# widdowquinn/pyani

Hardware: AMD Instinct MI355X
Metric: genome-pairs/sec (ordered pairs) + wall-clock for the N x N ANIm grid: nucmer --mum + delta-filter -1 + parse_delta equivalent per ordered pair, genomes resident in HBM; vs the CPU path on this box's host cores (higher is better)
Workload: dtype u32 packed DP words (score << 17 | state << 15 | errors), i64 lengths, f64 identity

## Files before the change

### pyani_amd/csrc/pg_nucmer_diag.h

```cpp
#pragma once
#include <stdint.h>
#include "pg_nucmer_core.h"

namespace pgd {
using namespace pgn;

template <int DPL> struct DiagRegs { uint32_t X[DPL], D[DPL], I[DPL], mw[DPL]; };

PG_HD uint32_t rev16_fields(uint32_t x) {
#if defined(__HIP_DEVICE_COMPILE__)
  x = __brev(x);
#else
  x = ((x >> 1) & 0x55555555u) | ((x & 0x55555555u) << 1);
  x = ((x >> 2) & 0x33333333u) | ((x & 0x33333333u) << 2);
  x = ((x >> 4) & 0x0F0F0F0Fu) | ((x & 0x0F0F0F0Fu) << 4);
  x = ((x >> 8) & 0x00FF00FFu) | ((x & 0x00FF00FFu) << 8);
  x = (x >> 16) | (x << 16);
#endif
  return ((x & 0x55555555u) << 1) | ((x >> 1) & 0x55555555u);
}
PG_HD uint32_t spread16(uint32_t m) {
  m &= 0xFFFFu;
  m = (m | (m << 8)) & 0x00FF00FFu;
  m = (m | (m << 4)) & 0x0F0F0F0Fu;
  m = (m | (m << 2)) & 0x33333333u;
  m = (m | (m << 1)) & 0x55555555u;
  return m;
}

struct DiagRelabel { uint32_t mask, st_insert, st_match; };
template <int DPL, int PAR, bool NORM = false>
PG_HD uint32_t diag_lane_edge(const DiagRegs<DPL>& T) {
  constexpr int32_t RISE = NORM && PAR == 0 ? GOOD_SCORE : 0;
  const uint32_t c = w_gap(PAR == 0 ? T.D[DPL - 1] : T.I[0], CONT_GAP_SCORE - RISE), x = w_gap(PAR == 0 ? T.X[DPL - 1] : T.X[0], OPEN_GAP_SCORE - RISE);
  return c > x ? c : x;
}
template <int DPL, int PAR, bool TRACK, bool NORM = false>
PG_HD void diag_lane_step(DiagRegs<DPL>& T, uint32_t nbM, uint32_t g0, uint32_t glo, uint32_t gspan, const DiagRelabel& rel,
                          uint32_t& key, uint32_t& keyw) {
  key = 0u; keyw = 0u;
  const uint32_t gofs = g0 - glo;
  constexpr int32_t RISE = NORM && PAR == 0 ? GOOD_SCORE : 0;
#if defined(__HIP_DEVICE_COMPILE__)
#pragma unroll
#endif
  for (int s = PAR; s < DPL; s += 2) {
    uint32_t dm, im;
    if (s == 0) dm = nbM;
    else { const uint32_t dc = w_gap(T.D[s - 1], CONT_GAP_SCORE - RISE), dx = w_gap(T.X[s - 1], OPEN_GAP_SCORE - RISE); dm = dc > dx ? dc : dx; }
    if (s == DPL - 1) im = nbM;
    else { const uint32_t ic = w_gap(T.I[s + 1], CONT_GAP_SCORE - RISE), ix = w_gap(T.X[s + 1], OPEN_GAP_SCORE - RISE); im = ic > ix ? ic : ix; }
    const bool in = (uint32_t)(gofs + (uint32_t)s) <= gspan;
    const uint32_t mk = in ? rel.mask : 0u;
    const uint32_t d = dm & mk , i = s == DPL - 1 ? (im & mk) + rel.st_insert : (im & mk) | rel.st_insert;
    const uint32_t m = ((NORM ? w_step_norm(T.X[s], T.mw[s]) : w_step_window(T.X[s], T.mw[s])) & mk) | rel.st_match;
    T.mw[s] <<= 2;
    T.X[s] = w_max3(d, i, m); T.D[s] = d; T.I[s] = i;
    if (TRACK) {
      const uint32_t k = (T.X[s] & ~(W_ONE - 1u)) | (g0 + (uint32_t)s);
      if (k >= key) { key = k; keyw = T.X[s]; }
    }
  }
}
template <int DPL, int PAR>
PG_HD void diag_lane_key(const DiagRegs<DPL>& T, uint32_t g0, uint32_t& key, uint32_t& keyw) {
  key = 0u; keyw = 0u;
#if defined(__HIP_DEVICE_COMPILE__)
#pragma unroll
#endif
  for (int s = PAR; s < DPL; s += 2) {
    const uint32_t k = (T.X[s] & ~(W_ONE - 1u)) | (g0 + (uint32_t)s);
    if (k >= key) { key = k; keyw = T.X[s]; }
  }
}
template <int DPL, int PAR>
PG_HD uint32_t diag_lane_top(const DiagRegs<DPL>& T) {
  uint32_t top = 0u;
#if defined(__HIP_DEVICE_COMPILE__)
#pragma unroll
#endif
  for (int s = PAR; s < DPL; s += 2) top = T.X[s] > top ? T.X[s] : top;
  return top;
}
template <int DPL, int PAR>
PG_HD uint32_t diag_lane_alive(const DiagRegs<DPL>& T, uint32_t thr) {
  uint32_t bits = 0u;
  for (int s = PAR; s < DPL; s += 2) bits |= (T.X[s] >= thr ? 1u : 0u) << s;
  return bits;
}
template <int DPL, int PAR, bool NORM = false, bool CLEAN = false>
PG_HD void diag_lane_refill(DiagRegs<DPL>& T, uint64_t ca, uint32_t oka, uint64_t cb, uint32_t okb) {
  constexpr int e_last = ((DPL - 1) ^ PAR) & 1, e_0 = PAR & 1;
#if defined(__HIP_DEVICE_COMPILE__)
#pragma unroll
#endif
  for (int s = 0; s < DPL; ++s) {
    const int e_s = (s ^ PAR) & 1;
    const int oa = (DPL - 1 - s + e_s - e_last) / 2, ob = (s + e_s - e_0) / 2;
    const uint32_t a16 = (uint32_t)(ca >> (2 * oa)), b16 = (uint32_t)(cb >> (2 * ob));
    const uint32_t x = a16 ^ b16;
    const uint32_t eq = ~(x | (x >> 1)) & 0x55555555u;
    const uint32_t hit = CLEAN ? eq : eq & spread16((oka >> oa) & (okb >> ob));
    T.mw[s] = rev16_fields(NORM ? hit ^ 0x55555555u : hit) << 1;
  }
}
template <int DPL, int PAR>
PG_HD void diag_refill_origin(int32_t Dct, int32_t k0, int32_t& ia0, int32_t& jb0) {
  constexpr int e_last = ((DPL - 1) ^ PAR) & 1, e_0 = PAR & 1;
  const int32_t u = Dct - k0;
  ia0 = (u - (DPL - 1) + e_last) >> 1;
  jb0 = ((u + e_0) >> 1) + k0;
}

struct DiagCtl {
  int32_t N, M, NM;
  bool fwd, forced, optimal, banded;
  int32_t Dct, Dend;
  int32_t ga, gb;
  int32_t lo, hi;
  int32_t c1g, c2g;
  int32_t kming, kmaxg;
  int32_t shiftk;
  uint32_t high_f, high_w;
  uint32_t high_fw, thr_w;
  int32_t FinishCt, FinishG, FinishShift;
  uint32_t span_sum;
  int32_t wmax;
  int32_t next_refill;
  template <int DPL>
  PG_HD void init(int32_t N_, int32_t M_, unsigned m_o, int32_t band_w) {
    constexpr int32_t HALF = 32 * DPL;
    N = N_; M = M_; NM = N_ + M_;
    fwd = m_o & DIRECTION_BIT; forced = m_o & FORCED_BIT; optimal = m_o & OPTIMAL_BIT; banded = band_w >= 0;
    kming = (M - N < 0 ? M - N : 0) - band_w + HALF; kmaxg = (M - N > 0 ? M - N : 0) + band_w + HALF;
    Dct = 1; Dend = forced ? NM : (NM < BREAK_LEN ? NM : BREAK_LEN);
    ga = HALF - 1; gb = HALF + 1; lo = HALF; hi = HALF; shiftk = 0;
    c1g = 1 - 2 * N + HALF; c2g = 2 * M - 1 + HALF;
    high_f = 0u; high_w = 0u; FinishCt = 0; FinishG = HALF; FinishShift = 0;
    high_fw = 0u; thr_w = (0u - (uint32_t)MAX_DIFF) << SCORE_SHIFT;
    span_sum = 0u; wmax = 0; next_refill = 1;
  }
  template <bool FORCED>
  PG_HD int begin_step() {
    if (Dct > Dend) return 1;
    lo = ga > c1g ? ga : c1g; hi = gb < c2g ? gb : c2g;
    if (FORCED && banded) {
      if (lo < kming) lo = kming;
      if (hi > kmaxg) hi = kmaxg;
      if ((lo + Dct) & 1) ++lo;
      if ((hi + Dct) & 1) --hi;
    }
    return lo > hi ? 2 : 0;
  }
  template <bool FORCED>
  PG_HD bool begin_step_go() {
    lo = ga > c1g ? ga : c1g; hi = gb < c2g ? gb : c2g;
    if (FORCED && banded) {
      if (lo < kming) lo = kming;
      if (hi > kmaxg) hi = kmaxg;
      if ((lo + Dct) & 1) ++lo;
      if ((hi + Dct) & 1) --hi;
    }
    return ((Dend - Dct) | (hi - lo)) >= 0;
  }
  template <int DPL>
  PG_HD int32_t window_check() const {
    constexpr int32_t W = 64 * DPL, HALF = W / 2;
    if (lo >= 2 && hi <= W - 3) return 0;
    if (hi - lo + 5 > W) return INT32_MIN;
    int32_t n = ((lo + hi) / 2 - HALF) / DPL;
    if (n == 0) n = lo < 2 ? -1 : 1;
    if (lo - DPL * n < 2 || hi - DPL * n > W - 3) return INT32_MIN;
    return n;
  }
  template <int DPL>
  PG_HD void window_move(int32_t n) { window_shift(DPL * n); }
  PG_HD void window_shift(int32_t d) {
    shiftk += d; lo -= d; hi -= d; ga -= d; gb -= d; c1g -= d; c2g -= d; kming -= d; kmaxg -= d;
    next_refill = Dct;
  }
  template <bool WIDEST>
  PG_HD void note_cells() {
    span_sum += (uint32_t)(hi - lo);
    if (WIDEST) { const int32_t w = (hi - lo) / 2 + 1; if (w > wmax) wmax = w; }
  }
  PG_HD int32_t steps() const { return Dct - 1; }
  PG_HD unsigned long long cells_total() const { return (unsigned long long)(span_sum / 2u) + (unsigned long long)steps(); }
  PG_HD void update_best(uint32_t gk, uint32_t gw) {
    const uint32_t f = gk >> SCORE_SHIFT;
    if (f >= (high_fw >> SCORE_SHIFT)) {
      high_f = f; high_w = gw; high_fw = f << SCORE_SHIFT; thr_w = (f - (uint32_t)MAX_DIFF) << SCORE_SHIFT; FinishCt = Dct; FinishG = (int32_t)(gk & (W_ONE - 1u)); FinishShift = shiftk;
      Dend = Dct + BREAK_LEN < NM ? Dct + BREAK_LEN : NM;
    }
  }
  PG_HD uint32_t trim_threshold() const { return thr_w; }
  template <bool FORCED, bool NORM_EVEN = false>
  PG_HD void end_step(bool any, uint32_t gmin, uint32_t gmax) {
    if (FORCED) { ga = lo - 1; gb = hi + 1; }
    else if (any) { ga = (int32_t)gmin - 1; gb = (int32_t)gmax + 1; }
    else { ga = 0; gb = 1; Dend = -1; }
    ++Dct; ++c1g; --c2g;
    if (NORM_EVEN) { high_fw -= (uint32_t)GOOD_SCORE << SCORE_SHIFT; thr_w -= (uint32_t)GOOD_SCORE << SCORE_SHIFT; }
  }
  template <int DPL>
  PG_HD bool finish1(bool& reached, uint32_t& corner_slot, int32_t& FinishK) {
    constexpr int32_t HALF = 32 * DPL;
    reached = false;
    const int32_t last = Dct - 1;
    corner_slot = 0u;
    FinishK = FinishG - HALF + FinishShift;
    if (last == NM) {
      if (!optimal) { reached = true; FinishCt = NM; FinishK = M - N; corner_slot = (uint32_t)(M - N - shiftk + HALF); return true; }
      if (FinishCt == last) reached = true;
    }
    return false;
  }
  template <bool NORM = false>
  PG_HD void finish2(uint32_t fin_w, int32_t FinishK, int32_t Astart, int32_t Bstart, int32_t& Aend, int32_t& Bend, int32_t& errors, int32_t& score) const {
    const int32_t fi = (FinishCt - FinishK) / 2, fj = (FinishCt + FinishK) / 2;
    Aend = fwd ? Astart + fi - 1 : Astart - fi + 1;
    Bend = fwd ? Bstart + fj - 1 : Bstart - fj + 1;
    errors = (int32_t)w_errors(fin_w);
    score = NORM ? (int32_t)(fin_w >> SCORE_SHIFT) - (int32_t)NORM_BIAS + norm_offset(FinishCt) : w_score(fin_w);
  }
};

#if !defined(__HIP_DEVICE_COMPILE__)
template <int DPL, typename RefT, typename QryT>
struct DiagWaveEmu {
  static constexpr int W = 64 * DPL, HALF = W / 2;
  const RefT& R;
  const QryT& Q;
  long cells = 0, calls = 0, moves = 0, fails = 0;
  uint32_t last_cells = 0, last_wmax = 0;
  DiagRegs<DPL> T[64];
  template <int PAR, bool NORM>
  void refill(const DiagCtl& C, int32_t Astart, int32_t Bstart) {
    for (int l = 0; l < 64; ++l) {
      const int32_t k0 = DPL * l - HALF + C.shiftk;
      int32_t ia0, jb0;
      diag_refill_origin<DPL, PAR>(C.Dct, k0, ia0, jb0);
      uint64_t ca = 0, cb = 0; uint32_t oka = 0, okb = 0;
      for (int f = 0; f < 32; ++f) {
        const int64_t pa = C.fwd ? (int64_t)Astart + (ia0 + f) - 1 : (int64_t)Astart - (ia0 + f) + 1;
        const int64_t pb = C.fwd ? (int64_t)Bstart + (jb0 + f) - 1 : (int64_t)Bstart - (jb0 + f) + 1;
        if (R.clean(pa)) { ca |= (uint64_t)R.base(pa) << (2 * f); oka |= 1u << f; }
        if (Q.clean(pb)) { cb |= (uint64_t)Q.base(pb) << (2 * f); okb |= 1u << f; }
      }
      if ((oka & okb) == 0xFFFFFFFFu) diag_lane_refill<DPL, PAR, NORM, true>(T[l], ca, oka, cb, okb);
      else diag_lane_refill<DPL, PAR, NORM, false>(T[l], ca, oka, cb, okb);
    }
  }
  template <int PAR, bool FORCED>
  void step(DiagCtl& C) {
    uint32_t nbM[64], key[64], keyw[64];
    for (int l = 0; l < 64; ++l) {
      if (PAR == 0) nbM[l] = l > 0 ? diag_lane_edge<DPL, PAR, !FORCED>(T[l - 1]) : 0u;
      else nbM[l] = l < 63 ? diag_lane_edge<DPL, PAR, !FORCED>(T[l + 1]) : 0u;
    }
    for (int l = 0; l < 64; ++l)
      diag_lane_step<DPL, PAR, !FORCED, !FORCED>(T[l], nbM[l], (uint32_t)(DPL * l), (uint32_t)C.lo, (uint32_t)(C.hi - C.lo), DiagRelabel{~W_STATE, ST_INSERT, ST_MATCH}, key[l], keyw[l]);
    bool any = false; uint32_t gmin = 0, gmax = 0;
    if (!FORCED) {
      uint32_t gk = 0, gw = 0;
      for (int l = 0; l < 64; ++l) if (key[l] > gk) { gk = key[l]; gw = keyw[l]; }
      C.update_best(gk, gw);
      const uint32_t thr = C.trim_threshold();
      for (int l = 0; l < 64; ++l) {
        const uint32_t bits = diag_lane_alive<DPL, PAR>(T[l], thr);
        for (int s = PAR; s < DPL; s += 2)
          if ((bits >> s) & 1u) { const uint32_t g = (uint32_t)(DPL * l + s); if (!any) { gmin = g; any = true; } gmax = g; }
      }
    }
    C.template end_step<FORCED, !FORCED && PAR == 1>(any, gmin, gmax);
  }
  template <bool FORCED>
  bool run_(int32_t Astart, int32_t& Aend, int32_t Bstart, int32_t& Bend, unsigned m_o, int32_t band_w, int32_t& errors, int32_t& score, bool& reached) {
    DiagCtl C;
    const bool fwd = m_o & DIRECTION_BIT;
    C.template init<DPL>(fwd ? Aend - Astart + 1 : Astart - Aend + 1, fwd ? Bend - Bstart + 1 : Bstart - Bend + 1, m_o, band_w);
    for (int l = 0; l < 64; ++l) for (int s = 0; s < DPL; ++s) { T[l].X[s] = 0u; T[l].D[s] = 0u; T[l].I[s] = 0u; T[l].mw[s] = 0u; }
    T[HALF / DPL].X[0] = FORCED ? w_make(0, 0, ST_MATCH) : (NORM_BIAS << SCORE_SHIFT) | ST_MATCH;
    ++calls;
    for (;;) {
      if (C.template begin_step<FORCED>()) break;
      const int32_t n = C.template window_check<DPL>();
      if (n == INT32_MIN) { ++fails; return false; }
      if (n != 0) {
        DiagRegs<DPL> Z;
        for (int s = 0; s < DPL; ++s) { Z.X[s] = 0u; Z.D[s] = 0u; Z.I[s] = 0u; Z.mw[s] = 0u; }
        DiagRegs<DPL> U[64];
        for (int l = 0; l < 64; ++l) U[l] = (l + n >= 0 && l + n < 64) ? T[l + n] : Z;
        for (int l = 0; l < 64; ++l) T[l] = U[l];
        C.template window_move<DPL>(n);
        ++moves;
      }
      if (C.Dct == C.next_refill) { if (C.Dct & 1) refill<1, !FORCED>(C, Astart, Bstart); else refill<0, !FORCED>(C, Astart, Bstart); C.next_refill = C.Dct + 32; }
      C.template note_cells<true>();
      if (C.Dct & 1) step<1, FORCED>(C); else step<0, FORCED>(C);
    }
    uint32_t corner = 0, fin_w = C.high_w;
    int32_t FinishK = 0;
    if (C.template finish1<DPL>(reached, corner, FinishK)) fin_w = T[corner / DPL].X[corner % DPL];
    C.template finish2<!FORCED>(fin_w, FinishK, Astart, Bstart, Aend, Bend, errors, score);
    const unsigned long long nc = C.cells_total();
    cells += (long)nc;
    last_cells = nc > 0xFFFFFFFFull ? 0xFFFFFFFFu : (uint32_t)nc; last_wmax = (uint32_t)C.wmax;
    return true;
  }
  bool run(int32_t Astart, int32_t& Aend, int32_t Bstart, int32_t& Bend, unsigned m_o, int32_t band_w, int32_t& errors, int32_t& score, bool& reached) {
    return (m_o & FORCED_BIT) ? run_<true>(Astart, Aend, Bstart, Bend, m_o, band_w, errors, score, reached)
                              : run_<false>(Astart, Aend, Bstart, Bend, m_o, band_w, errors, score, reached);
  }
};
#endif

PG_HD bool diag_window_holds(int64_t span, int dpl) { return span <= 64 * (int64_t)dpl - 2 * (int64_t)dpl + 2; }
#if !defined(__HIP_DEVICE_COMPILE__)
template <typename RefT, typename QryT>
struct DiagWaveEngine {
  ScalarEngine<RefT, QryT> slow;
  DiagWaveEmu<2, RefT, QryT> e2;
  DiagWaveEmu<4, RefT, QryT> e4;
  DiagWaveEmu<6, RefT, QryT> e6;
  DiagWaveEmu<8, RefT, QryT> e8;
  DiagWaveEmu<12, RefT, QryT> e12;
  DiagWaveEmu<16, RefT, QryT> e16;
  DiagWaveEmu<24, RefT, QryT> e24;
  DiagWaveEmu<32, RefT, QryT> e32;
  long fallbacks = 0;
  void (*fallback_log)(int32_t N, int32_t M, unsigned m_o, int32_t band_w) = nullptr;
  DiagWaveEngine(const RefT& R, const QryT& Q, Cell* d0, Cell* d1, Cell* d2, int32_t cap)
      : slow{R, Q, d0, d1, d2, cap}, e2{R, Q}, e4{R, Q}, e6{R, Q}, e8{R, Q}, e12{R, Q}, e16{R, Q}, e24{R, Q}, e32{R, Q} {}
  bool gap_ready(int32_t, PnGap&) const { return false; }
  void piece(uint32_t, int32_t, int32_t, int32_t, int32_t, int32_t, int32_t, int32_t, unsigned) {}
  bool bwd_ready(int, PnBwd&) const { return false; }
  void bwd_key(int, int32_t, int32_t, int32_t, int32_t, unsigned) {}
  bool fwd_ready(int, PnFwd&) const { return false; }
  int32_t forced_errors(int32_t A0, int32_t A1, int32_t B0, int32_t B1, PnAln*) {
    int32_t err = 0, a = A1, b = B1;
    align(A0, a, B0, b, FORCED_FORWARD_ALIGN, err);
    return err;
  }
  bool shadowed(const Chain* chains, const PnAln* al, int from, int c, int32_t sA, int32_t eA, int32_t sB, int32_t eB) const {
    return PnScalarScans().shadowed(chains, al, from, c, sA, eA, sB, eB); }
  int shadow_first(const Chain* chains, const PnAln* al, int n_al, int c, int32_t sA, int32_t eA, int32_t sB, int32_t eB) const {
    return PnScalarScans().shadow_first(chains, al, n_al, c, sA, eA, sB, eB); }
  int reverse_target(const Chain* chains, const PnAln* al, int cura, int c, int32_t sA, int32_t sB, int32_t dist) const {
    return PnScalarScans().reverse_target(chains, al, cura, c, sA, sB, dist); }
  int forward_target(const Chain* chains, const Match* cm, const int32_t* order, int n, int curk, int c, int32_t sA, int32_t sB,
                     int32_t dist, int32_t& targetA, int32_t& targetB) const {
    return PnScalarScans().forward_target(chains, cm, order, n, curk, c, sA, sB, dist, targetA, targetB); }
  static int window_for(int32_t N, int32_t M, unsigned m_o, int32_t band_w) {
    if (!(m_o & FORCED_BIT)) return 256;
    const int32_t df = N < M ? M - N : N - M;
    const int64_t span = band_w >= 0 ? (int64_t)df + 2 * (int64_t)band_w + 1 : (int64_t)N + M + 1;
    for (int w : {128, 256, 384, 512, 768, 1024, 1536, 2048}) if (diag_window_holds(span + 5, w / 64)) return w;
    return 0;
  }
  bool run(int32_t Astart, int32_t& Aend, int32_t Bstart, int32_t& Bend, unsigned m_o, int32_t band_w, int32_t& errors, int32_t& score) {
    const bool fwd = m_o & DIRECTION_BIT;
    const int32_t N = fwd ? Aend - Astart + 1 : Astart - Aend + 1, M = fwd ? Bend - Bstart + 1 : Bstart - Bend + 1;
    int32_t a = Aend, b = Bend;
    bool reached = false, done = false;
    switch (window_for(N, M, m_o, band_w)) {
      case 128: done = e2.run(Astart, a, Bstart, b, m_o, band_w, errors, score, reached); break;
      case 256: done = e4.run(Astart, a, Bstart, b, m_o, band_w, errors, score, reached); break;
      case 384: done = e6.run(Astart, a, Bstart, b, m_o, band_w, errors, score, reached); break;
      case 512: done = e8.run(Astart, a, Bstart, b, m_o, band_w, errors, score, reached); break;
      case 768: done = e12.run(Astart, a, Bstart, b, m_o, band_w, errors, score, reached); break;
      case 1024: done = e16.run(Astart, a, Bstart, b, m_o, band_w, errors, score, reached); break;
      case 1536: done = e24.run(Astart, a, Bstart, b, m_o, band_w, errors, score, reached); break;
      case 2048: done = e32.run(Astart, a, Bstart, b, m_o, band_w, errors, score, reached); break;
      default: break;
    }
    if (done) { Aend = a; Bend = b; return reached; }
    ++fallbacks;
    if (fallback_log) fallback_log(N, M, m_o, band_w);
    return slow.run(Astart, Aend, Bstart, Bend, m_o, band_w, errors, &score);
  }
  bool align(int32_t Astart, int32_t& Aend, int32_t Bstart, int32_t& Bend, unsigned m_o, int32_t& errors) {
    int32_t score = 0;
    if (!(m_o & FORCED_BIT)) return run(Astart, Aend, Bstart, Bend, m_o, -1, errors, score);
    const bool fwd = m_o & DIRECTION_BIT;
    const int32_t N = fwd ? Aend - Astart + 1 : Astart - Aend + 1, M = fwd ? Bend - Bstart + 1 : Bstart - Bend + 1;
    for (int32_t w = FORCED_BAND_FIRST;;) {
      int32_t a = Aend, b = Bend;
      const bool whole = w >= (N > M ? N : M);
      const bool reached = run(Astart, a, Bstart, b, m_o, whole ? -1 : w, errors, score);
      const int v = slow.overflow ? 0 : forced_verdict(reached, score, whole, N, M, w);
      if (v == 2) { slow.overflow = 1; Aend = a; Bend = b; errors = 0; return false; }
      if (v == 0) { Aend = a; Bend = b; return reached; }
      w = forced_band_after(w, N, M, score);
    }
  }
};
#endif

}
```

### pyani_amd/csrc/pga_postnuc_diag.inc

```

__device__ __forceinline__ void strand_window(const StrandView& Q, int64_t p0, uint64_t& c, uint32_t& ok) {
  if (!Q.rc) { packed_window(Q.s.codes, Q.s.mask, (int32_t)Q.s.len, p0, c, ok); return; }
  uint64_t w; uint32_t k;
  packed_window(Q.s.codes, Q.s.mask, (int32_t)Q.s.len, Q.s.len - 32 - p0, w, k);
  const uint32_t lo = rev_fields2((uint32_t)(w >> 32)), hi = rev_fields2((uint32_t)w);
  c = ~(((uint64_t)hi << 32) | lo);
  ok = __brev(k);
}
__device__ __forceinline__ void rev_window32(uint64_t& c, uint32_t& ok) {
  const uint32_t lo = rev_fields2((uint32_t)(c >> 32)), hi = rev_fields2((uint32_t)c);
  c = ((uint64_t)hi << 32) | lo;
  ok = __brev(ok);
}
struct PnRawWin { uint32_t c0, c1, c2, m0, m1; };
__device__ __forceinline__ PnRawWin packed_window_load(const uint32_t* __restrict__ codes, const uint32_t* __restrict__ mask, int32_t len, int64_t p0) {
  const bool out = p0 >= len || p0 + 32 <= 0;
  const int64_t q0 = out ? 0 : (p0 < 0 ? 0 : p0);
  const int32_t w = (int32_t)(q0 >> 4), lastw = len > 0 ? (len - 1) >> 4 : 0;
  const int32_t mw = (int32_t)(q0 >> 5), lastm = len > 0 ? (len - 1) >> 5 : 0;
  PnRawWin r;
  r.c0 = codes[w]; r.c1 = codes[w + 1 <= lastw ? w + 1 : lastw]; r.c2 = codes[w + 2 <= lastw ? w + 2 : lastw];
  r.m0 = mask[mw]; r.m1 = mask[mw + 1 <= lastm ? mw + 1 : lastm];
  return r;
}
__device__ __forceinline__ void packed_window_finish(const PnRawWin& r, int32_t len, int64_t p0, uint64_t& c, uint32_t& ok) {
  const bool out = p0 >= len || p0 + 32 <= 0;
  const int64_t q0 = out ? 0 : (p0 < 0 ? 0 : p0);
  const int sh = out ? 0 : (int)(q0 - p0);
  const int cs = 2 * (int)(q0 & 15);
  const uint64_t lo = ((uint64_t)r.c1 << 32) | r.c0;
  const uint64_t win = (lo >> cs) | (cs ? (uint64_t)r.c2 << ((64 - cs) & 63) : 0ull);
  const uint64_t m = ((uint64_t)r.m1 << 32) | r.m0;
  uint32_t okw = (uint32_t)(m >> (q0 & 31));
  const int64_t avail = len - q0;
  okw &= avail < 32 ? (1u << (avail & 31)) - 1u : 0xFFFFFFFFu;
  c = out ? 0ull : win << (2 * sh);
  ok = out ? 0u : okw << sh;
}
struct PnRefillPos { int64_t pa, pb; };
template <int DPL, int PAR, int HALF = 32 * DPL>
__device__ __forceinline__ PnRefillPos pn_diag_refill_pos(const StrandView& Q, const pgd::DiagCtl& C, int32_t Dct, int32_t Astart, int32_t Bstart, int lane) {
  const int32_t k0 = DPL * lane - HALF + C.shiftk;
  int32_t ia0, jb0;
  pgd::diag_refill_origin<DPL, PAR>(Dct, k0, ia0, jb0);
  PnRefillPos P;
  P.pa = C.fwd ? (int64_t)Astart + ia0 - 1 : (int64_t)Astart - ia0 - 30;
  const int64_t sb = C.fwd ? (int64_t)Bstart + jb0 - 1 : (int64_t)Bstart - jb0 - 30;
  P.pb = Q.rc ? Q.s.len - 32 - sb : sb;
  return P;
}
template <int DPL, int PAR, int HALF = 32 * DPL, bool NORM = false>
__device__ __forceinline__ void pn_diag_refill(pgd::DiagRegs<DPL>& T, const SeqView& R, const StrandView& Q, const pgd::DiagCtl& C,
                                               int32_t Astart, int32_t Bstart, int lane, PnRawWin& na, PnRawWin& nb, bool& have_next) {
  const PnRefillPos P = pn_diag_refill_pos<DPL, PAR, HALF>(Q, C, C.Dct, Astart, Bstart, lane);
  if (!have_next) { na = packed_window_load(R.codes, R.mask, (int32_t)R.len, P.pa); nb = packed_window_load(Q.s.codes, Q.s.mask, (int32_t)Q.s.len, P.pb); }
  uint64_t ca, cb; uint32_t oka, okb;
  packed_window_finish(na, (int32_t)R.len, P.pa, ca, oka);
  packed_window_finish(nb, (int32_t)Q.s.len, P.pb, cb, okb);
  if (Q.rc) { rev_window32(cb, okb); cb = ~cb; }
  if (!C.fwd) { rev_window32(ca, oka); rev_window32(cb, okb); }
  if (__ballot((oka & okb) != 0xFFFFFFFFu) == 0ull) pgd::diag_lane_refill<DPL, PAR, NORM, true>(T, ca, oka, cb, okb);
  else pgd::diag_lane_refill<DPL, PAR, NORM, false>(T, ca, oka, cb, okb);
  const PnRefillPos N = pn_diag_refill_pos<DPL, PAR, HALF>(Q, C, C.Dct + 32, Astart, Bstart, lane);
  na = packed_window_load(R.codes, R.mask, (int32_t)R.len, N.pa);
  nb = packed_window_load(Q.s.codes, Q.s.mask, (int32_t)Q.s.len, N.pb);
  have_next = true;
}

template <int YES>
__device__ __forceinline__ int pn_bit_select(uint64_t m, int b, int no) {
  int r;
  asm("s_bitcmp1_b64 %1, %2\n\ts_cselect_b32 %0, %3, %4" : "=s"(r) : "s"(m), "s"(b), "n"(YES), "s"(no) : "scc");
  return r;
}
template <int YES, int NO>
__device__ __forceinline__ int pn_bit_select2(uint64_t m, int b) {
  int r;
  asm("s_bitcmp1_b64 %1, %2\n\ts_cselect_b32 %0, %3, %4" : "=s"(r) : "s"(m), "s"(b), "n"(YES), "n"(NO) : "scc");
  return r;
}
template <int PAR>
__device__ __forceinline__ int pn_bit_select_t(int t, uint64_t m, int b, int no) {
  switch (t) {
#define PN_CASE(T_) case T_: return pn_bit_select<PAR + 2 * T_>(m, b, no);
    PN_CASE(0) PN_CASE(1) PN_CASE(2) PN_CASE(3) PN_CASE(4) PN_CASE(5) PN_CASE(6) PN_CASE(7)
    PN_CASE(8) PN_CASE(9) PN_CASE(10) PN_CASE(11) PN_CASE(12) PN_CASE(13) PN_CASE(14) PN_CASE(15)
#undef PN_CASE
  }
  return no;
}
template <int DPL, int PAR, bool FORCED>
__device__ __forceinline__ void pn_diag_step(pgd::DiagRegs<DPL>& T, pgd::DiagCtl& C, int lane, const pgd::DiagRelabel& relmask) {
  using namespace pgd;
  const uint32_t edge = diag_lane_edge<DPL, PAR, !FORCED>(T);
  const uint32_t nbM = PAR == 0 ? dpp_from_below0(edge) : dpp_from_above0(edge);
  uint32_t key, keyw;
  diag_lane_step<DPL, PAR, false, !FORCED>(T, nbM, (uint32_t)(DPL * lane), (uint32_t)C.lo, (uint32_t)(C.hi - C.lo), relmask, key, keyw);
  bool any = false;
  uint32_t gmin = 0u, gmax = 0u;
  if constexpr (!FORCED) {
    if (__ballot(diag_lane_top<DPL, PAR>(T) >= C.high_fw) != 0ull) {
      diag_lane_key<DPL, PAR>(T, (uint32_t)(DPL * lane), key, keyw);
      const uint32_t gk = wave_max_u32(key);
      const uint64_t who = __ballot(key == gk);
      const uint32_t gw = (uint32_t)__builtin_amdgcn_readlane((int)keyw, __builtin_amdgcn_readfirstlane((int)__builtin_ctzll(who)));
      C.update_best(gk, gw);
    }
    const uint32_t thr = C.trim_threshold();
    uint64_t m[DPL / 2], all = 0ull;
#pragma unroll
    for (int t = 0; t < DPL / 2; ++t) { m[t] = __ballot(T.X[PAR + 2 * t] >= thr); all |= m[t]; }
    any = all != 0ull;
    if (any) {
      const int l0 = (int)__builtin_ctzll(all), l1 = 63 - (int)__builtin_clzll(all);
      int s0 = pn_bit_select2<PAR + DPL - 4, PAR + DPL - 2>(m[DPL / 2 - 2], l0), s1 = pn_bit_select2<PAR + 2, PAR>(m[1], l1);
#pragma unroll
      for (int t = DPL / 2 - 3; t >= 0; --t) s0 = pn_bit_select_t<PAR>(t, m[t], l0, s0);
#pragma unroll
      for (int t = 2; t < DPL / 2; ++t) s1 = pn_bit_select_t<PAR>(t, m[t], l1, s1);
      gmin = (uint32_t)(DPL * l0 + s0); gmax = (uint32_t)(DPL * l1 + s1);
    }
  }
  C.template end_step<FORCED, !FORCED && PAR == 1>(any, gmin, gmax);
}

template <int DPL, int PAR, bool FORCED, bool INFO>
__device__ __forceinline__ bool pn_diag_advance(pgd::DiagRegs<DPL>& T, pgd::DiagCtl& C, const SeqView& R, const StrandView& Q, int32_t Astart,
                                                int32_t Bstart, int lane, uint32_t& stat_moves, const pgd::DiagRelabel& relmask,
                                                PnRawWin& na, PnRawWin& nb, bool& have_next) {
  constexpr int32_t W = 64 * DPL;
  if (!C.template begin_step_go<FORCED>()) return false;
  if (__builtin_expect(((C.lo - 2) | (W - 3 - C.hi)) < 0, 0)) {
    const int32_t n = C.template window_check<DPL>();
    if (n == INT32_MIN) { C.Dend = INT32_MIN; return false; }
#pragma unroll
    for (int s = 0; s < DPL; ++s) {
      const int src = lane + n;
      const uint32_t x = (uint32_t)__shfl((int)T.X[s], src & 63, 64), d = (uint32_t)__shfl((int)T.D[s], src & 63, 64), i = (uint32_t)__shfl((int)T.I[s], src & 63, 64);
      const bool ok = src >= 0 && src < 64;
      T.X[s] = ok ? x : 0u; T.D[s] = ok ? d : 0u; T.I[s] = ok ? i : 0u;
    }
    C.template window_move<DPL>(n);
    ++stat_moves;
    have_next = false;
  }
  if (C.Dct == C.next_refill) { pn_diag_refill<DPL, PAR, 32 * DPL, !FORCED>(T, R, Q, C, Astart, Bstart, lane, na, nb, have_next); C.next_refill = C.Dct + 32; }
  C.template note_cells<INFO>();
  pn_diag_step<DPL, PAR, FORCED>(T, C, lane, relmask);
  return true;
}

template <int DPL, bool FORCED, bool INFO>
__device__ bool pn_align_diag_run(const SeqView& R_, const StrandView& Q_, int32_t Astart_, int32_t& Aend, int32_t Bstart_, int32_t& Bend,
                                  unsigned m_o_, int32_t band_w_, int32_t& errors, int32_t& score, bool& reached, PnRunInfo* info,
                                  int kstat) {
  using namespace pgd;
  constexpr int32_t HALF = 32 * DPL;
  const int lane = threadIdx.x & 63;
  const SeqView R = pn_uni(R_);
  const StrandView Q = pn_uni(Q_);
  const int32_t Astart = pn_uni(Astart_), Bstart = pn_uni(Bstart_), Aend0 = pn_uni(Aend), Bend0 = pn_uni(Bend);
  const unsigned m_o = pn_uni((uint32_t)m_o_);
  const bool fwd = m_o & DIRECTION_BIT;
  DiagCtl C;
  C.template init<DPL>(fwd ? Aend0 - Astart + 1 : Astart - Aend0 + 1, fwd ? Bend0 - Bstart + 1 : Bstart - Bend0 + 1, m_o, pn_uni(band_w_));
  DiagRegs<DPL> T;
#pragma unroll
  for (int s = 0; s < DPL; ++s) { T.X[s] = 0u; T.D[s] = 0u; T.I[s] = 0u; T.mw[s] = 0u; }
  if (lane == HALF / DPL) T.X[0] = FORCED ? w_make(0, 0, ST_MATCH) : (NORM_BIAS << SCORE_SHIFT) | ST_MATCH;
  uint32_t stat_moves = 0;
  DiagRelabel relmask;
  asm volatile("v_mov_b32 %0, 0xfffe7fff" : "=v"(relmask.mask));
  asm volatile("v_mov_b32 %0, 0x8000" : "=v"(relmask.st_insert));
  asm volatile("v_mov_b32 %0, 0x10000" : "=v"(relmask.st_match));
  PnRawWin na{0u, 0u, 0u, 0u, 0u}, nb{0u, 0u, 0u, 0u, 0u};
  bool have_next = false;
  for (;;) {
    if (!pn_diag_advance<DPL, 1, FORCED, INFO>(T, C, R, Q, Astart, Bstart, lane, stat_moves, relmask, na, nb, have_next)) break;
    if (!pn_diag_advance<DPL, 0, FORCED, INFO>(T, C, R, Q, Astart, Bstart, lane, stat_moves, relmask, na, nb, have_next)) break;
  }
  {
    const uint32_t keep = (uint32_t)(C.ga ^ C.gb ^ C.lo ^ C.hi ^ C.c1g ^ C.c2g ^ C.next_refill) ^ C.high_fw ^ C.thr_w;
    asm volatile("" ::"s"(keep));
  }
  if (C.Dend == INT32_MIN) { pn_stat(10, 1); return false; }
  const unsigned long long cells = C.cells_total();
  if (info) { info->cells = cells; info->wmax = C.wmax; }
  pn_stat(0, 1); pn_stat(1, (unsigned long long)C.steps()); pn_stat(2, cells); pn_stat(9, stat_moves);
  if (kstat >= 0) pn_kstat(kstat, 1ull, (unsigned long long)C.steps(), cells);
  uint32_t corner = 0u, fin_w = C.high_w;
  bool rch = false;
  int32_t FinishK = 0;
  if (C.template finish1<DPL>(rch, corner, FinishK)) {
    const int src = __builtin_amdgcn_readfirstlane((int)(corner / DPL));
    const uint32_t cs = corner % DPL;
    uint32_t v = 0u;
#pragma unroll
    for (int s = 0; s < DPL; ++s) if (cs == (uint32_t)s) v = T.X[s];
    fin_w = (uint32_t)__builtin_amdgcn_readlane((int)v, src);
  }
  reached = rch;
  C.template finish2<!FORCED>(fin_w, FinishK, Astart, Bstart, Aend, Bend, errors, score);
  return true;
}
template <int DPL>
__device__ __forceinline__ bool pn_align_diag(const SeqView& R, const StrandView& Q, int32_t Astart, int32_t& Aend, int32_t Bstart, int32_t& Bend,
                                              unsigned m_o, int32_t band_w, int32_t& errors, int32_t& score, bool& reached, PnRunInfo* info = nullptr,
                                              int kstat = -1) {
  if (pn_uni((uint32_t)m_o) & pgn::FORCED_BIT) return pn_align_diag_run<DPL, true, false>(R, Q, Astart, Aend, Bstart, Bend, m_o, band_w, errors, score, reached, info, kstat);
  if constexpr (DPL < 4) return false;
  else {
    if (info) return pn_align_diag_run<DPL, false, true>(R, Q, Astart, Aend, Bstart, Bend, m_o, band_w, errors, score, reached, info, kstat);
    return pn_align_diag_run<DPL, false, false>(R, Q, Astart, Aend, Bstart, Bend, m_o, band_w, errors, score, reached, info, kstat);
  }
}

template <int NW, int DPL>
__device__ bool pn_forced_diag_group(const SeqView& R_, const StrandView& Q_, int32_t A0_, int32_t A1_, int32_t B0_, int32_t B1_, int32_t band_w_,
                                     uint32_t* xch, int32_t& errors, int32_t& score, int kstat) {
  using namespace pgd;
  constexpr int DPLE = DPL * NW, W = 64 * DPLE, HALF = W / 2;
  const int lane = threadIdx.x & 63, wave = __builtin_amdgcn_readfirstlane((int)(threadIdx.x >> 6)), glane = 64 * wave + lane;
  const SeqView R = pn_uni(R_);
  const StrandView Q = pn_uni(Q_);
  const int32_t A0 = pn_uni(A0_), A1 = pn_uni(A1_), B0 = pn_uni(B0_), B1 = pn_uni(B1_), band_w = pn_uni(band_w_);
  DiagCtl C;
  C.template init<DPLE>(A1 - A0 + 1, B1 - B0 + 1, FORCED_FORWARD_ALIGN, band_w);
  {
    const int32_t klo = band_w >= 0 ? C.kming - HALF : -C.N, khi = band_w >= 0 ? C.kmaxg - HALF : C.M;
    C.window_shift(2 * ((klo + khi) / 4));
    if (klo - C.shiftk + HALF < 2 || khi - C.shiftk + HALF > W - 3) return false;
  }
  DiagRegs<DPL> T;
#pragma unroll
  for (int s = 0; s < DPL; ++s) { T.X[s] = 0u; T.D[s] = 0u; T.I[s] = 0u; T.mw[s] = 0u; }
  {
    const int32_t g = 0 - C.shiftk + HALF;
#pragma unroll
    for (int s = 0; s < DPL; ++s) if (glane == g / DPL && (g % DPL) == s) T.X[s] = w_make(0, 0, ST_MATCH);
  }
  DiagRelabel rel;
  asm volatile("v_mov_b32 %0, 0xfffe7fff" : "=v"(rel.mask));
  asm volatile("v_mov_b32 %0, 0x8000" : "=v"(rel.st_insert));
  asm volatile("v_mov_b32 %0, 0x10000" : "=v"(rel.st_match));
  PnRawWin na{0u, 0u, 0u, 0u, 0u}, nb{0u, 0u, 0u, 0u, 0u};
  bool have_next = false;
  int why = 0, buf = 0;
  while (!why) {
    why = C.template begin_step<true>();
    if (!why && (C.lo < 2 || C.hi > W - 3)) why = 3;
    if (why) break;
    const int par = C.Dct & 1;
    if (C.Dct == C.next_refill) {
      if (par) pn_diag_refill<DPL, 1, HALF>(T, R, Q, C, A0, B0, glane, na, nb, have_next); else pn_diag_refill<DPL, 0, HALF>(T, R, Q, C, A0, B0, glane, na, nb, have_next);
      C.next_refill = C.Dct + 32;
    }
    C.template note_cells<false>();
    uint32_t* mine = xch + (buf * NW + wave) * 4;
    const uint32_t edge = par == 0 ? diag_lane_edge<DPL, 0>(T) : diag_lane_edge<DPL, 1>(T);
    if (par == 0) { if (lane == 63) mine[0] = edge; }
    else { if (lane == 0) mine[2] = edge; }
    __syncthreads();
    uint32_t key, keyw;
    if (par == 0) {
      uint32_t nbM = dpp_from_below0(edge);
      if (lane == 0 && wave > 0) nbM = xch[(buf * NW + wave - 1) * 4];
      diag_lane_step<DPL, 0, false>(T, nbM, (uint32_t)(DPL * glane), (uint32_t)C.lo, (uint32_t)(C.hi - C.lo), rel, key, keyw);
    } else {
      uint32_t nbM = dpp_from_above0(edge);
      if (lane == 63 && wave + 1 < NW) nbM = xch[(buf * NW + wave + 1) * 4 + 2];
      diag_lane_step<DPL, 1, false>(T, nbM, (uint32_t)(DPL * glane), (uint32_t)C.lo, (uint32_t)(C.hi - C.lo), rel, key, keyw);
    }
    C.template end_step<true>(false, 0u, 0u);
    buf ^= 1;
  }
  if (why == 3) return false;
  const unsigned long long cells = C.cells_total();
  if (wave == 0) { pn_stat(0, 1); pn_stat(1, (unsigned long long)C.steps()); pn_stat(2, cells); if (kstat >= 0) pn_kstat(kstat, 1ull, (unsigned long long)C.steps(), cells); }
  uint32_t corner = 0u, fin_w = C.high_w;
  bool rch = false;
  int32_t FinishK = 0;
  uint32_t* res = xch + 2 * NW * 4;
  __syncthreads();
  if (C.template finish1<DPLE>(rch, corner, FinishK)) {
#pragma unroll
    for (int s = 0; s < DPL; ++s) if (glane == (int)(corner / DPL) && (corner % DPL) == (uint32_t)s) res[0] = T.X[s];
    __syncthreads();
    fin_w = res[0];
  }
  if (!rch) return false;
  int32_t a = A1, b = B1;
  C.finish2(fin_w, FinishK, A0, B0, a, b, errors, score);
  __syncthreads();
  return true;
}
```

Measured before the change: 65150.

## Batch provably-safe diagonal steps to skip per-step bounds, window and refill checks

Adds a safe-run mode to the diagonal DP: after each full step it computes how many upcoming antidiagonals cannot hit the band edges, need a window shift, need a refill or reach Dend. Those steps then run with lighter begin/end bookkeeping (no c1g/c2g updates, no window check, deferred best/Dend update) and are committed in end_run. Only the FORCED path uses it on device. This trims per-step scalar control overhead at the cost of more code and a host emulator cross-check counter.

```diff
diff --git a/pyani_amd/csrc/pg_nucmer_diag.h b/pyani_amd/csrc/pg_nucmer_diag.h
--- a/pyani_amd/csrc/pg_nucmer_diag.h
+++ b/pyani_amd/csrc/pg_nucmer_diag.h
@@ -127,6 +127,9 @@
   uint32_t span_sum;
   int32_t wmax;
   int32_t next_refill;
+  int32_t run_D0;
+  uint32_t best_key;
+  int32_t lo_floor[2], hi_ceil[2];
   template <int DPL>
   PG_HD void init(int32_t N_, int32_t M_, unsigned m_o, int32_t band_w) {
     constexpr int32_t HALF = 32 * DPL;
@@ -202,6 +205,49 @@
     ++Dct; ++c1g; --c2g;
     if (NORM_EVEN) { high_fw -= (uint32_t)GOOD_SCORE << SCORE_SHIFT; thr_w -= (uint32_t)GOOD_SCORE << SCORE_SHIFT; }
   }
+
+  template <int DPL>
+  PG_HD int32_t safe_steps() const {
+    constexpr int32_t W = 64 * DPL;
+    int32_t s = 32;
+    const int32_t a = ((ga - c1g) >> 1) + 1, b = ((c2g - gb) >> 1) + 1, c = ga - 1, d = W - 2 - gb, e = next_refill - Dct, f = Dend - Dct + 1;
+    s = a < s ? a : s; s = b < s ? b : s; s = c < s ? c : s; s = d < s ? d : s; s = e < s ? e : s; s = f < s ? f : s;
+    return s > 0 ? s : 0;
+  }
+  PG_HD void open_run() {
+    run_D0 = Dct;
+    if (forced && banded) {
+      lo_floor[0] = kming + (kming & 1); lo_floor[1] = kming + ((kming + 1) & 1);
+      hi_ceil[0] = kmaxg - (kmaxg & 1); hi_ceil[1] = kmaxg - ((kmaxg + 1) & 1);
+    } else { lo_floor[0] = lo_floor[1] = INT32_MIN; hi_ceil[0] = hi_ceil[1] = INT32_MAX; }
+  }
+  template <bool FORCED, int PAR>
+  PG_HD void begin_step_safe() {
+    if (FORCED) { lo = ga > lo_floor[PAR] ? ga : lo_floor[PAR]; hi = gb < hi_ceil[PAR] ? gb : hi_ceil[PAR]; }
+    else { lo = ga; hi = gb; }
+  }
+  PG_HD void update_best_run(uint32_t gk, uint32_t gw) {
+    const uint32_t f = gk >> SCORE_SHIFT;
+    if (f >= (high_fw >> SCORE_SHIFT)) {
+      best_key = gk; high_w = gw; high_fw = f << SCORE_SHIFT; thr_w = (f - (uint32_t)MAX_DIFF) << SCORE_SHIFT; FinishCt = Dct;
+    }
+  }
+  template <bool FORCED, bool NORM_EVEN = false>
+  PG_HD void end_step_safe(bool any, uint32_t gmin, uint32_t gmax) {
+    if (FORCED) { ga = lo - 1; gb = hi + 1; }
+    else if (any) { ga = (int32_t)gmin - 1; gb = (int32_t)gmax + 1; }
+    else { ga = 0; gb = 1; Dend = -1; }
+    ++Dct;
+    if (NORM_EVEN) { high_fw -= (uint32_t)GOOD_SCORE << SCORE_SHIFT; thr_w -= (uint32_t)GOOD_SCORE << SCORE_SHIFT; }
+  }
+  PG_HD void end_run() {
+    const int32_t n = Dct - run_D0;
+    c1g += n; c2g -= n;
+    if (FinishCt >= run_D0) {
+      high_f = best_key >> SCORE_SHIFT; FinishG = (int32_t)(best_key & (W_ONE - 1u)); FinishShift = shiftk;
+      if (Dend >= 0) Dend = FinishCt + BREAK_LEN < NM ? FinishCt + BREAK_LEN : NM;
+    }
+  }
   template <int DPL>
   PG_HD bool finish1(bool& reached, uint32_t& corner_slot, int32_t& FinishK) {
     constexpr int32_t HALF = 32 * DPL;
@@ -232,6 +278,7 @@
   const RefT& R;
   const QryT& Q;
   long cells = 0, calls = 0, moves = 0, fails = 0;
+  long steps = 0, safe = 0, safe_bad = 0;
   uint32_t last_cells = 0, last_wmax = 0;
   DiagRegs<DPL> T[64];
   template <int PAR, bool NORM>
@@ -251,8 +298,8 @@
       else diag_lane_refill<DPL, PAR, NORM, false>(T[l], ca, oka, cb, okb);
     }
   }
-  template <int PAR, bool FORCED>
-  void step(DiagCtl& C) {
+  template <int PAR, bool FORCED, bool SAFE = false>
+  bool step(DiagCtl& C) {
     uint32_t nbM[64], key[64], keyw[64];
     for (int l = 0; l < 64; ++l) {
       if (PAR == 0) nbM[l] = l > 0 ? diag_lane_edge<DPL, PAR, !FORCED>(T[l - 1]) : 0u;
@@ -264,7 +311,7 @@
     if (!FORCED) {
       uint32_t gk = 0, gw = 0;
       for (int l = 0; l < 64; ++l) if (key[l] > gk) { gk = key[l]; gw = keyw[l]; }
-      C.update_best(gk, gw);
+      if (SAFE) C.update_best_run(gk, gw); else C.update_best(gk, gw);
       const uint32_t thr = C.trim_threshold();
       for (int l = 0; l < 64; ++l) {
         const uint32_t bits = diag_lane_alive<DPL, PAR>(T[l], thr);
@@ -272,7 +319,55 @@
           if ((bits >> s) & 1u) { const uint32_t g = (uint32_t)(DPL * l + s); if (!any) { gmin = g; any = true; } gmax = g; }
       }
     }
-    C.template end_step<FORCED, !FORCED && PAR == 1>(any, gmin, gmax);
+    if (SAFE) C.template end_step_safe<FORCED, !FORCED && PAR == 1>(any, gmin, gmax);
+    else C.template end_step<FORCED, !FORCED && PAR == 1>(any, gmin, gmax);
+    return FORCED || any;
+  }
+  template <bool FORCED>
+  int full_step(DiagCtl& C, int32_t Astart, int32_t Bstart) {
+    if (C.template begin_step<FORCED>()) return 1;
+    const int32_t n = C.template window_check<DPL>();
+    if (n == INT32_MIN) return 2;
+    if (n != 0) {
+      DiagRegs<DPL> Z;
+      for (int s = 0; s < DPL; ++s) { Z.X[s] = 0u; Z.D[s] = 0u; Z.I[s] = 0u; Z.mw[s] = 0u; }
+      DiagRegs<DPL> U[64];
+      for (int l = 0; l < 64; ++l) U[l] = (l + n >= 0 && l + n < 64) ? T[l + n] : Z;
+      for (int l = 0; l < 64; ++l) T[l] = U[l];
+      C.template window_move<DPL>(n);
+      ++moves;
+    }
+    if (C.Dct == C.next_refill) { if (C.Dct & 1) refill<1, !FORCED>(C, Astart, Bstart); else refill<0, !FORCED>(C, Astart, Bstart); C.next_refill = C.Dct + 32; }
+    C.template note_cells<true>();
+    if (C.Dct & 1) step<1, FORCED>(C); else step<0, FORCED>(C);
+    return 0;
+  }
+  template <int PAR, bool FORCED>
+  bool safe_step(DiagCtl& C) {
+    {
+      DiagCtl F = C;
+      F.end_run(); F.run_D0 = F.Dct;
+      const int why = F.template begin_step<FORCED>();
+      DiagCtl G = C;
+      G.template begin_step_safe<FORCED, PAR>();
+      if ((C.Dct & 1) != PAR || why != 0 || F.lo != G.lo || F.hi != G.hi || F.template window_check<DPL>() != 0 || F.Dct == F.next_refill) ++safe_bad;
+    }
+    C.template begin_step_safe<FORCED, PAR>();
+    C.template note_cells<true>();
+    ++safe;
+    return step<PAR, FORCED, true>(C);
+  }
+  template <int PAR0, bool FORCED>
+  void safe_run(DiagCtl& C) {
+    constexpr int PAR1 = PAR0 ^ 1;
+    const int32_t S = C.template safe_steps<DPL>() & ~1;
+    C.open_run();
+    const int32_t Dstop = C.Dct + S;
+    bool alive = true;
+    while (alive && C.Dct + 4 <= Dstop)
+      alive = safe_step<PAR0, FORCED>(C) && safe_step<PAR1, FORCED>(C) && safe_step<PAR0, FORCED>(C) && safe_step<PAR1, FORCED>(C);
+    if (alive && C.Dct + 2 <= Dstop) alive = safe_step<PAR0, FORCED>(C) && safe_step<PAR1, FORCED>(C);
+    C.end_run();
   }
   template <bool FORCED>
   bool run_(int32_t Astart, int32_t& Aend, int32_t Bstart, int32_t& Bend, unsigned m_o, int32_t band_w, int32_t& errors, int32_t& score, bool& reached) {
@@ -282,22 +377,11 @@
     for (int l = 0; l < 64; ++l) for (int s = 0; s < DPL; ++s) { T[l].X[s] = 0u; T[l].D[s] = 0u; T[l].I[s] = 0u; T[l].mw[s] = 0u; }
     T[HALF / DPL].X[0] = FORCED ? w_make(0, 0, ST_MATCH) : (NORM_BIAS << SCORE_SHIFT) | ST_MATCH;
     ++calls;
-    for (;;) {
-      if (C.template begin_step<FORCED>()) break;
-      const int32_t n = C.template window_check<DPL>();
-      if (n == INT32_MIN) { ++fails; return false; }
-      if (n != 0) {
-        DiagRegs<DPL> Z;
-        for (int s = 0; s < DPL; ++s) { Z.X[s] = 0u; Z.D[s] = 0u; Z.I[s] = 0u; Z.mw[s] = 0u; }
-        DiagRegs<DPL> U[64];
-        for (int l = 0; l < 64; ++l) U[l] = (l + n >= 0 && l + n < 64) ? T[l + n] : Z;
-        for (int l = 0; l < 64; ++l) T[l] = U[l];
-        C.template window_move<DPL>(n);
-        ++moves;
-      }
-      if (C.Dct == C.next_refill) { if (C.Dct & 1) refill<1, !FORCED>(C, Astart, Bstart); else refill<0, !FORCED>(C, Astart, Bstart); C.next_refill = C.Dct + 32; }
-      C.template note_cells<true>();
-      if (C.Dct & 1) step<1, FORCED>(C); else step<0, FORCED>(C);
+    for (int why = 0;;) {
+      if ((why = full_step<FORCED>(C, Astart, Bstart)) != 0) { if (why == 2) { ++fails; return false; } break; }
+      if (FORCED) safe_run<0, FORCED>(C);
+      if ((why = full_step<FORCED>(C, Astart, Bstart)) != 0) { if (why == 2) { ++fails; return false; } break; }
+      if (FORCED) safe_run<1, FORCED>(C);
     }
     uint32_t corner = 0, fin_w = C.high_w;
     int32_t FinishK = 0;
@@ -305,6 +389,7 @@
     C.template finish2<!FORCED>(fin_w, FinishK, Astart, Bstart, Aend, Bend, errors, score);
     const unsigned long long nc = C.cells_total();
     cells += (long)nc;
+    steps += (long)C.steps();
     last_cells = nc > 0xFFFFFFFFull ? 0xFFFFFFFFu : (uint32_t)nc; last_wmax = (uint32_t)C.wmax;
     return true;
   }
diff --git a/pyani_amd/csrc/pga_postnuc_diag.inc b/pyani_amd/csrc/pga_postnuc_diag.inc
--- a/pyani_amd/csrc/pga_postnuc_diag.inc
+++ b/pyani_amd/csrc/pga_postnuc_diag.inc
@@ -89,8 +89,8 @@
   }
   return no;
 }
-template <int DPL, int PAR, bool FORCED>
-__device__ __forceinline__ void pn_diag_step(pgd::DiagRegs<DPL>& T, pgd::DiagCtl& C, int lane, const pgd::DiagRelabel& relmask) {
+template <int DPL, int PAR, bool FORCED, bool SAFE = false>
+__device__ __forceinline__ bool pn_diag_step(pgd::DiagRegs<DPL>& T, pgd::DiagCtl& C, int lane, const pgd::DiagRelabel& relmask) {
   using namespace pgd;
   const uint32_t edge = diag_lane_edge<DPL, PAR, !FORCED>(T);
   const uint32_t nbM = PAR == 0 ? dpp_from_below0(edge) : dpp_from_above0(edge);
@@ -104,7 +104,7 @@
       const uint32_t gk = wave_max_u32(key);
       const uint64_t who = __ballot(key == gk);
       const uint32_t gw = (uint32_t)__builtin_amdgcn_readlane((int)keyw, __builtin_amdgcn_readfirstlane((int)__builtin_ctzll(who)));
-      C.update_best(gk, gw);
+      if constexpr (SAFE) C.update_best_run(gk, gw); else C.update_best(gk, gw);
     }
     const uint32_t thr = C.trim_threshold();
     uint64_t m[DPL / 2], all = 0ull;
@@ -121,7 +121,9 @@
       gmin = (uint32_t)(DPL * l0 + s0); gmax = (uint32_t)(DPL * l1 + s1);
     }
   }
-  C.template end_step<FORCED, !FORCED && PAR == 1>(any, gmin, gmax);
+  if constexpr (SAFE) C.template end_step_safe<FORCED, !FORCED && PAR == 1>(any, gmin, gmax);
+  else C.template end_step<FORCED, !FORCED && PAR == 1>(any, gmin, gmax);
+  return FORCED || any;
 }
 
 template <int DPL, int PAR, bool FORCED, bool INFO>
@@ -148,6 +150,31 @@
   C.template note_cells<INFO>();
   pn_diag_step<DPL, PAR, FORCED>(T, C, lane, relmask);
   return true;
+}
+
+template <int DPL, int PAR, bool FORCED, bool INFO>
+__device__ __forceinline__ bool pn_diag_safe(pgd::DiagRegs<DPL>& T, pgd::DiagCtl& C, int lane, const pgd::DiagRelabel& relmask) {
+  C.template begin_step_safe<FORCED, PAR>();
+  C.template note_cells<INFO>();
+  return pn_diag_step<DPL, PAR, FORCED, true>(T, C, lane, relmask);
+}
+template <int DPL, int PAR0, bool FORCED, bool INFO>
+__device__ __forceinline__ void pn_diag_safe_steps(pgd::DiagRegs<DPL>& T, pgd::DiagCtl& C, int lane, const pgd::DiagRelabel& relmask, int32_t Dstop) {
+  constexpr int PAR1 = PAR0 ^ 1;
+  while (C.Dct + 4 <= Dstop) {
+    if (!pn_diag_safe<DPL, PAR0, FORCED, INFO>(T, C, lane, relmask)) return;
+    if (!pn_diag_safe<DPL, PAR1, FORCED, INFO>(T, C, lane, relmask)) return;
+    if (!pn_diag_safe<DPL, PAR0, FORCED, INFO>(T, C, lane, relmask)) return;
+    if (!pn_diag_safe<DPL, PAR1, FORCED, INFO>(T, C, lane, relmask)) return;
+  }
+  if (C.Dct + 2 <= Dstop && pn_diag_safe<DPL, PAR0, FORCED, INFO>(T, C, lane, relmask)) pn_diag_safe<DPL, PAR1, FORCED, INFO>(T, C, lane, relmask);
+}
+template <int DPL, int PAR0, bool FORCED, bool INFO>
+__device__ __forceinline__ void pn_diag_safe_run(pgd::DiagRegs<DPL>& T, pgd::DiagCtl& C, int lane, const pgd::DiagRelabel& relmask) {
+  const int32_t Dstop = C.Dct + (C.template safe_steps<DPL>() & ~1);
+  C.open_run();
+  pn_diag_safe_steps<DPL, PAR0, FORCED, INFO>(T, C, lane, relmask, Dstop);
+  C.end_run();
 }
 
 template <int DPL, bool FORCED, bool INFO>
@@ -175,9 +202,18 @@
   asm volatile("v_mov_b32 %0, 0x10000" : "=v"(relmask.st_match));
   PnRawWin na{0u, 0u, 0u, 0u, 0u}, nb{0u, 0u, 0u, 0u, 0u};
   bool have_next = false;
-  for (;;) {
-    if (!pn_diag_advance<DPL, 1, FORCED, INFO>(T, C, R, Q, Astart, Bstart, lane, stat_moves, relmask, na, nb, have_next)) break;
-    if (!pn_diag_advance<DPL, 0, FORCED, INFO>(T, C, R, Q, Astart, Bstart, lane, stat_moves, relmask, na, nb, have_next)) break;
+  if constexpr (FORCED) {
+    for (;;) {
+      if (!pn_diag_advance<DPL, 1, FORCED, INFO>(T, C, R, Q, Astart, Bstart, lane, stat_moves, relmask, na, nb, have_next)) break;
+      pn_diag_safe_run<DPL, 0, FORCED, INFO>(T, C, lane, relmask);
+      if (!pn_diag_advance<DPL, 0, FORCED, INFO>(T, C, R, Q, Astart, Bstart, lane, stat_moves, relmask, na, nb, have_next)) break;
+      pn_diag_safe_run<DPL, 1, FORCED, INFO>(T, C, lane, relmask);
+    }
+  } else {
+    for (;;) {
+      if (!pn_diag_advance<DPL, 1, FORCED, INFO>(T, C, R, Q, Astart, Bstart, lane, stat_moves, relmask, na, nb, have_next)) break;
+      if (!pn_diag_advance<DPL, 0, FORCED, INFO>(T, C, R, Q, Astart, Bstart, lane, stat_moves, relmask, na, nb, have_next)) break;
+    }
   }
   {
     const uint32_t keep = (uint32_t)(C.ga ^ C.gb ^ C.lo ^ C.hi ^ C.c1g ^ C.c2g ^ C.next_refill) ^ C.high_fw ^ C.thr_w;
```

Result: no change. 65760, median of 6 (+0.9%).
